# visinf/style-seqcvae

Measured on AMD Instinct MI355X. Metric: captions/sec (train step), higher is better.
Workload: dtype f32; 1 GPU; C2 train step: fwd+bwd+allreduce+clip+SGD, B=64/GPU, R=36, F=2048, L=20 (T=21), Z=128, V=10000, E=1000, H=1200, A=768, SENTIMENT_VAE=1; global_batch=64, parallelism=dp1

## Files before the change

### include/ssc.h

```cpp
#ifndef SSC_H
#define SSC_H

#include <stddef.h>
#include <stdint.h>

#ifdef __cplusplus
extern "C" {
#endif

#define SSC_OK 0
#define SSC_EINVAL (-1)
#define SSC_EALIGN (-2)
#define SSC_EHIP (-3)
#define SSC_EWORKSPACE (-4)

#define SSC_MAX_SEG 6

int ssc_version(void);
int ssc_last_hip_error(void);
const char* ssc_arch(void);

typedef struct {
  const float* A; const float* B;
  int lda, ldb, K;
// ... 72 lines not shown
  const float* c_prev; int ld_cprev;
  const float* c_new; int ld_cnew;
  float* dG;
  float* dc_prev; int ld_dcprev;
  float* dgsum;
  const float* slabsA; int nA; size_t strideA;
  const float* slabsB; int nB; size_t strideB;
} ssc_lstm_bwd_desc;
int ssc_lstm_bwd(const ssc_lstm_bwd_desc* d, void* stream);
int ssc_lstm_bwd_x(const ssc_lstm_bwd_desc* d, const float* x, int ldx, const float* w, int ldw, int K, void* stream);

int ssc_attn_logits(const float* q, int ldq, const float* pv, const float* wa, int G, int R, int A, int rows_per_image,
                    float* logits, void* stream);
int ssc_attn_fwd(const float* q, int ldq, const float* pv, const float* wa, const float* mask, const float* feats,
                 int G, int R, int A, int F, int rows_per_image, float* logits, float* alpha, float* att, int ldatt,
                 void* stream);

int ssc_attn_weights(const float* q, int ldq, const float* pv, const float* wa, const float* mask, int G, int R, int A,
                     int rows_per_image, float* logits, float* alpha, void* stream);

int ssc_attn_pool(const float* alpha, const float* x, int G, int R, int D, int rows_per_image, float* out, int ldo,
                  void* stream);
int ssc_attn_fwd_pool(const float* q, int ldq, const float* pv, const float* wa, const float* mask, const float* feats,
                      int G, int R, int A, int F, int rows_per_image, float* logits, float* alpha, float* att, int ldatt,
                      const float* obj, int D, float* pool, int ldpool, void* stream);

int ssc_attn_bwd(const float* datt, int lddatt, const float* q, int ldq, const float* pv, const float* wa,
                 const float* alpha, const float* feats, int G, int R, int A, int F, float* dq, int lddq,
                 float* dpv_acc, float* dwa_acc, float* scratch_dalpha, void* stream);
int ssc_attn_bwd_pool(const float* datt, int lddatt, const float* q, int ldq, const float* pv, const float* wa,
                      const float* alpha, const float* feats, int G, int R, int A, int F, float* dq, int lddq,
                      float* dpv_acc, float* dwa_acc, float* scratch_dalpha, const float* obj, int D, const float* dpool_a,
                      int lddpa, int Da, const float* dpool_b, int lddpb, void* stream);

typedef struct {
  int B, Z;
  const float* mulv; int ldmulv; int nslab; size_t slab_stride;
  const float* bmu; const float* blv;
  const float* eps; int ldeps;
  int kld_mode;
  const float* sent; float pm_scale; float prior_var;
  const float* w;
  float* mu; float* lv; float* z; int ldz;
  float* kld_acc;
  const float* pm; int ldpm;
} ssc_latent_fwd_desc;
int ssc_latent_fwd(const ssc_latent_fwd_desc* d, void* stream);

int ssc_latent_prior_sample(const float* eps, int ldeps, const float* sent, float pm_scale, float prior_var, int G, int Z,
                            float* z, int ldz, void* stream);

int ssc_latent_prior_sample_pm(const float* eps, int ldeps, const float* pm, int ldpm, const float* pv, int ldpv, const float* sent,
                               float pm_scale, float prior_var, int G, int Z, float* z, int ldz, void* stream);

typedef struct {
  int B, Z;
  const float* dz; int lddz;
  const float* eps; int ldeps;
  const float* mu; const float* lv; int ldz;
  int kld_mode; const float* sent; float pm_scale; float prior_var;
  const float* w; const float* gk;
  float* dmulv; int lddmulv;
  int nslab; size_t slab_stride;
  const float* pm; int ldpm;
  float* dpm; int lddpm;
} ssc_latent_bwd_desc;
// ... 389 lines not shown
```

### style-seqcvae_amd/csrc/attention.hip

```cpp
#include "ssc_common.h"

namespace {

constexpr int ATTN_RG = 8;
constexpr int ATTN_MAXA = 4096;
__global__ __launch_bounds__(256) void attn_logits_kernel(const float* __restrict__ q, int ldq, int nslab, size_t slab_stride,
                                                          float* __restrict__ q_out, int ldqo,
                                                          const float* __restrict__ pv, const float* __restrict__ wa,
                                                          int G, int R, int A, int rows_per_image,
                                                          float* __restrict__ logits, const int* __restrict__ rows,
                                                          const int* __restrict__ row_count) {
  __shared__ __attribute__((aligned(16))) float sq[ATTN_MAXA];
  const int groups = (R + ATTN_RG - 1) / ATTN_RG;
  int g = blockIdx.x / groups;
  const int grp = blockIdx.x - g * groups;
  if (rows) {
    if (g >= *row_count) return;
    g = rows[g];
  }
  const int tid = threadIdx.x, wave = tid >> 6, lane = tid & 63;
  const int img = g / rows_per_image;
  const float* qp = q + (size_t)g * ldq;
  const bool vec = ((A & 3) == 0) && ((ldq & 3) == 0) && ((ldqo & 3) == 0) && ((slab_stride & 3) == 0) && ssc_aligned16_dev(qp) &&
                   ssc_aligned16_dev(pv) && ssc_aligned16_dev(wa) && (!q_out || ssc_aligned16_dev(q_out));
// ... 181 lines not shown
  out[(size_t)g * ldo + d] = acc;
}

__global__ __launch_bounds__(256) void attn_dalpha_kernel(const float* __restrict__ datt, int lddatt,
                                                          const float* __restrict__ feats, int G, int R, int F,
                                                          float* __restrict__ dalpha, const float* __restrict__ obj, int D,
                                                          const float* __restrict__ dpa, int lddpa, int Da,
                                                          const float* __restrict__ dpb, int lddpb) {
  int wid = blockIdx.x * 4 + (threadIdx.x >> 6);
  int lane = threadIdx.x & 63;
  if (wid >= G * R) return;
  int g = wid / R;
  const float* dp = datt + (size_t)g * lddatt;
  const float* fp = feats + (size_t)wid * F;
  float s = 0.f;
  if (((F & 3) == 0) && ((lddatt & 3) == 0) && ssc_aligned16_dev(dp) && ssc_aligned16_dev(fp)) {
    for (int f = lane * 4; f < F; f += 256) {
      float4 a = *reinterpret_cast<const float4*>(dp + f);
      float4 b = *reinterpret_cast<const float4*>(fp + f);
      s += a.x * b.x + a.y * b.y + a.z * b.z + a.w * b.w;
    }
  } else {
    for (int f = lane; f < F; f += 64) s += dp[f] * fp[f];
  }
  if (obj) {
    const float* op = obj + (size_t)wid * D;
    for (int k = lane; k < D; k += 64)
      s += ((k < Da ? dpa[(size_t)g * lddpa + k] : 0.f) + (dpb ? dpb[(size_t)g * lddpb + k] : 0.f)) * op[k];
  }
  s = ssc_wave_sum(s);
  if (lane == 0) dalpha[wid] = s;
}

__global__ __launch_bounds__(256) void attn_bwd_apply_kernel(const float* __restrict__ q, int ldq,
                                                             const float* __restrict__ pv, const float* __restrict__ wa,
                                                             const float* __restrict__ alpha,
                                                             const float* __restrict__ dalpha, int G, int R, int A,
                                                             float* __restrict__ dq, int lddq, float* __restrict__ dpv_acc,
                                                             float* __restrict__ dwa_acc) {
  __shared__ float sdl[64 * MAXR_LANE];
  __shared__ float red[2][4][256];
  const int g = blockIdx.y, chunk = blockIdx.x, tid = threadIdx.x, lane = tid & 63, wave = tid >> 6;
  float c = 0.f;
  for (int r = lane; r < R; r += 64) c += alpha[(size_t)g * R + r] * dalpha[(size_t)g * R + r];
  c = ssc_wave_sum(c);
  if (wave == 0)
    for (int r = lane; r < R; r += 64) sdl[r] = alpha[(size_t)g * R + r] * (dalpha[(size_t)g * R + r] - c);
  __syncthreads();
  const int a0 = chunk * 256 + lane * 4;
  float dqa[4] = {0.f, 0.f, 0.f, 0.f}, dw[4] = {0.f, 0.f, 0.f, 0.f};
  const bool vec = ((A & 3) == 0) && ((ldq & 3) == 0) && ssc_aligned16_dev(q) && ssc_aligned16_dev(pv) &&
                   ssc_aligned16_dev(wa) && ssc_aligned16_dev(dpv_acc);
  if (vec) {
    if (a0 < A) {
      const float4 qv = *reinterpret_cast<const float4*>(q + (size_t)g * ldq + a0);
      const float4 wv = *reinterpret_cast<const float4*>(wa + a0);
      const float qa[4] = {qv.x, qv.y, qv.z, qv.w}, ww[4] = {wv.x, wv.y, wv.z, wv.w};
      for (int rb = wave; rb < R; rb += 4 * 5) {
        float4 p4[5], ac[5];
#pragma unroll
        for (int i = 0; i < 5; ++i) {
          const size_t off = ((size_t)g * R + min(rb + 4 * i, R - 1)) * A + a0;
          p4[i] = *reinterpret_cast<const float4*>(pv + off);
          ac[i] = *reinterpret_cast<const float4*>(dpv_acc + off);
        }
#pragma unroll
        for (int i = 0; i < 5; ++i) {
          const int r = rb + 4 * i;
          if (r < R) {
            const float pp[4] = {p4[i].x, p4[i].y, p4[i].z, p4[i].w};
            float dp[4];
            const float dl = sdl[r];
#pragma unroll
            for (int k = 0; k < 4; ++k) {
              float u = ssc_tanh_fast(qa[k] + pp[k]);
              dp[k] = dl * ww[k] * (1.f - u * u);
              dqa[k] += dp[k];
              dw[k] += dl * u;
            }
            float4 acc = ac[i];
            acc.x += dp[0]; acc.y += dp[1]; acc.z += dp[2]; acc.w += dp[3];
            *reinterpret_cast<float4*>(dpv_acc + ((size_t)g * R + r) * A + a0) = acc;
          }
        }
      }
    }
  } else {
    for (int k = 0; k < 4; ++k) {
      int a = chunk * 256 + k * 64 + lane;
      if (a >= A) continue;
      float qa = q[(size_t)g * ldq + a], w = wa[a];
      for (int r = wave; r < R; r += 4) {
        size_t off = ((size_t)g * R + r) * A + a;
        float u = ssc_tanh_fast(qa + pv[off]);
        float dl = sdl[r];
        float dpre = dl * w * (1.f - u * u);
        dpv_acc[off] += dpre;
        dqa[k] += dpre;
        dw[k] += dl * u;
      }
    }
  }
#pragma unroll
  for (int k = 0; k < 4; ++k) {
    red[0][wave][lane * 4 + k] = dqa[k];
    red[1][wave][lane * 4 + k] = dw[k];
  }
  __syncthreads();
  {
    float s0 = red[0][0][tid] + red[0][1][tid] + red[0][2][tid] + red[0][3][tid];
    float s1 = red[1][0][tid] + red[1][1][tid] + red[1][2][tid] + red[1][3][tid];
    int l = tid >> 2, k = tid & 3;
    int a = vec ? (chunk * 256 + l * 4 + k) : (chunk * 256 + k * 64 + l);
    if (a < A) {
      dq[(size_t)g * lddq + a] = s0;
      dwa_acc[(size_t)g * A + a] += s1;
    }
  }
}

}

extern "C" int ssc_attn_logits(const float* q, int ldq, const float* pv, const float* wa, int G, int R, int A,
                               int rows_per_image, float* logits, void* stream) {
  if (!q || !pv || !wa || !logits || G <= 0 || R <= 0 || A <= 0 || A > ATTN_MAXA || rows_per_image <= 0 || ldq < A) return SSC_EINVAL;
  SSC_LAUNCH(attn_logits_kernel, dim3(G * ssc_cdiv(R, ATTN_RG)), dim3(256), 0, (hipStream_t)stream, q, ldq, 1, (size_t)0,
                     (float*)nullptr, 0, pv, wa, G, R, A, rows_per_image, logits, (const int*)nullptr, (const int*)nullptr);
  SSC_CHECK_LAUNCH();
  return SSC_OK;
}

int ssc_attn_weights_rows(const float* q, int ldq, const float* pv, const float* wa, const float* mask, int G, int R, int A,
                          int rows_per_image, float* logits, float* alpha, const int* rows, const int* row_count, hipStream_t st) {
  if (!q || !pv || !wa || !mask || !alpha || !logits || !rows || !row_count || G <= 0 || R <= 0 || A <= 0 || A > ATTN_MAXA ||
      rows_per_image <= 0 || ldq < A || R > 64 * MAXR_LANE)
    return SSC_EINVAL;
  SSC_LAUNCH(attn_logits_kernel, dim3(G * ssc_cdiv(R, ATTN_RG)), dim3(256), 0, st, q, ldq, 1, (size_t)0, (float*)nullptr, 0, pv, wa,
             G, R, A, rows_per_image, logits, rows, row_count);
  SSC_CHECK_LAUNCH();
  SSC_LAUNCH(attn_apply_kernel, dim3(1, G), dim3(64), 0, st, logits, mask, (const float*)nullptr, G, R, 4, rows_per_image, alpha,
             (float*)nullptr, 0, (const float*)nullptr, 0, (float*)nullptr, 0);
  SSC_CHECK_LAUNCH();
  return SSC_OK;
}

extern "C" int ssc_attn_fwd(const float* q, int ldq, const float* pv, const float* wa, const float* mask,
                            const float* feats, int G, int R, int A, int F, int rows_per_image, float* logits,
                            float* alpha, float* att, int ldatt, void* stream) {
  if (!mask || !feats || !alpha || !att || !logits || F <= 0 || ldatt < F) return SSC_EINVAL;
  if (R > 64 * MAXR_LANE) return SSC_EINVAL;
  SSC_TRY(ssc_attn_logits(q, ldq, pv, wa, G, R, A, rows_per_image, logits, stream));
  SSC_LAUNCH(attn_apply_kernel, dim3(ssc_cdiv(F, 256), G), dim3(64), 0, (hipStream_t)stream, logits, mask, feats,
                     G, R, F, rows_per_image, alpha, att, ldatt, (const float*)nullptr, 0, (float*)nullptr, 0);
// ... 30 lines not shown
  SSC_LAUNCH(attn_pool_kernel, dim3(ssc_cdiv((D + 3) & ~3, 128), G), dim3(128), 0, (hipStream_t)stream, alpha, x, G, R, D, rows_per_image,
             out, ldo);
  SSC_CHECK_LAUNCH();
  return SSC_OK;
}

int ssc_attn_fwd_qslabs(const float* qslabs, int nslab, size_t slab_stride, float* q_out, int ldqo, const float* pv,
                        const float* wa, const float* mask, const float* feats, int G, int R, int A, int F,
                        int rows_per_image, float* logits, float* alpha, float* att, int ldatt, hipStream_t st,
                        const float* obj, int D, float* pool, int ldpool) {
  if (!qslabs || nslab < 1 || !q_out || !pv || !wa || !mask || !feats || !alpha || !att || !logits) return SSC_EINVAL;
  if (obj && (!pool || D <= 0 || ldpool < D)) return SSC_EINVAL;
  if (G <= 0 || R <= 0 || A <= 0 || A > ATTN_MAXA || F <= 0 || ldatt < F || ldqo < A || R > 64 * MAXR_LANE) return SSC_EINVAL;
  SSC_LAUNCH(attn_logits_kernel, dim3(G * ssc_cdiv(R, ATTN_RG)), dim3(256), 0, st, qslabs, A, nslab, slab_stride, q_out,
                     ldqo, pv, wa, G, R, A, rows_per_image, logits, (const int*)nullptr, (const int*)nullptr);
  SSC_CHECK_LAUNCH();
  SSC_LAUNCH(attn_apply_kernel, dim3(ssc_cdiv(F, 256) + (obj ? ssc_cdiv(ldpool, 256) : 0), G), dim3(64), 0, st, logits, mask, feats,
             G, R, F, rows_per_image, alpha, att, ldatt, obj, D, pool, ldpool);
  SSC_CHECK_LAUNCH();
  return SSC_OK;
}

extern "C" int ssc_attn_bwd(const float* datt, int lddatt, const float* q, int ldq, const float* pv, const float* wa,
                            const float* alpha, const float* feats, int G, int R, int A, int F, float* dq, int lddq,
                            float* dpv_acc, float* dwa_acc, float* scratch_dalpha, void* stream) {
  return ssc_attn_bwd_pool(datt, lddatt, q, ldq, pv, wa, alpha, feats, G, R, A, F, dq, lddq, dpv_acc, dwa_acc, scratch_dalpha,
                           nullptr, 0, nullptr, 0, 0, nullptr, 0, stream);
}

extern "C" int ssc_attn_bwd_pool(const float* datt, int lddatt, const float* q, int ldq, const float* pv, const float* wa,
                                 const float* alpha, const float* feats, int G, int R, int A, int F, float* dq, int lddq,
                                 float* dpv_acc, float* dwa_acc, float* scratch_dalpha, const float* obj, int D,
                                 const float* dpool_a, int lddpa, int Da, const float* dpool_b, int lddpb, void* stream) {
  if (!datt || !q || !pv || !wa || !alpha || !feats || !dq || !dpv_acc || !dwa_acc || !scratch_dalpha) return SSC_EINVAL;
  if (G <= 0 || R <= 0 || A <= 0 || F <= 0 || R > 64 * MAXR_LANE || lddatt < F || ldq < A || lddq < A) return SSC_EINVAL;
  if (obj && (!dpool_a || D <= 0 || Da < 0 || Da > D || lddpa < Da || (dpool_b && lddpb < D))) return SSC_EINVAL;
  SSC_LAUNCH(attn_dalpha_kernel, dim3(ssc_cdiv(G * R, 4)), dim3(256), 0, (hipStream_t)stream, datt, lddatt, feats,
                     G, R, F, scratch_dalpha, obj, D, dpool_a, lddpa, Da, dpool_b, lddpb);
  SSC_CHECK_LAUNCH();
  SSC_LAUNCH(attn_bwd_apply_kernel, dim3(ssc_cdiv(A, 256), G), dim3(256), 0, (hipStream_t)stream, q, ldq, pv, wa,
                     alpha, scratch_dalpha, G, R, A, dq, lddq, dpv_acc, dwa_acc);
  SSC_CHECK_LAUNCH();
  return SSC_OK;
}
```

### style-seqcvae_amd/csrc/gemm.hip

```cpp
#include <stdio.h>
#include <stdlib.h>
#include <string.h>

#include "ssc_common.h"
#include "ssc_debug.h"

typedef float f32x16 __attribute__((ext_vector_type(16)));

namespace {

constexpr int BM = 64, BN = 64, BK = 32;
constexpr int KC_LD = BK + 4;

struct KSeg {
  const float* A;
  const float* B;
  int lda, ldb, K, nsteps;
  int avec, bvec;
  const float* A16;
  const float* B16;
  int lda16, ldb16;
};

struct KArgs {
// ... 2221 lines not shown
extern "C" int ssc_prof_collect(float* out, int max_records) {
  if (!out || !g_prof) return 0;
  if (hipDeviceSynchronize() != hipSuccess) return SSC_EHIP;
  int n = g_prof_n < max_records ? g_prof_n : max_records;
  for (int i = 0; i < n; ++i) {
    float ms = 0.f;
    (void)hipEventElapsedTime(&ms, g_prof[i].e0, g_prof[i].e1);
    float* o = out + (size_t)i * 8;
    g_prof[i].bytes = g_prof[i].flops = 0.0;
    for (int q = 0; q < g_prof[i].nmem; ++q) {
      const ProfMember& m = g_prof[i].mem[q];
      double M = m.M, K = m.K;
      if (m.slot_m >= 0 && g_prof_counts[m.slot_m] >= 0 && g_prof_counts[m.slot_m] < m.M) M = g_prof_counts[m.slot_m];
      if (m.slot_k >= 0 && g_prof_counts[m.slot_k] >= 0 && g_prof_counts[m.slot_k] < m.K) K = g_prof_counts[m.slot_k];
      g_prof[i].bytes += 4.0 * (K * m.N + M * K + M * m.N);
      g_prof[i].flops += 2.0 * M * m.N * K;
    }
    o[0] = (float)g_prof[i].kind; o[1] = (float)g_prof[i].M; o[2] = (float)g_prof[i].N; o[3] = (float)g_prof[i].K;
    o[4] = (float)g_prof[i].splits; o[5] = ms; o[6] = (float)g_prof[i].bytes; o[7] = (float)g_prof[i].flops;
  }
  g_prof_n = 0;
  g_prof_slots = 0;
  return n;
}

extern "C" int ssc_set_gemm_mode(int mode) {
  int prev = gemm_mode();
  if (mode == 0 || mode == 1) g_gemm_mode = mode;
  return prev;
}

extern int ssc_g_dec_att_table, ssc_g_dec_dedup, ssc_g_beam_reg, ssc_g_dec_ungathered, ssc_g_dec_parts, ssc_g_dec_planes;
extern int ssc_g_img_mfma;
extern int ssc_g_dw_one_flush;
namespace {
struct DebugKey { const char* name; int* var; };
const DebugKey g_debug_keys[] = {
    {"large_form", &g_x3b},
    {"x3w_skinny", &g_x3w_skinny},
    {"store_wt", &g_store_wt},
    {"tile_gm", &g_tile_gm},
    {"dw_one_flush", &ssc_g_dw_one_flush},
    {"dec_dedup", &ssc_g_dec_dedup},
    {"beam_reg", &ssc_g_beam_reg},
    {"img_mfma", &ssc_g_img_mfma},
    {"dec_ungathered", &ssc_g_dec_ungathered},
    {"dec_planes", &ssc_g_dec_planes},
    {"dec_parts", &ssc_g_dec_parts},
    {"dec_att_table", &ssc_g_dec_att_table},
    {"f16_npw", &g_f16_npw},
    {"gemm_f16", &g_gemm_f16},
};
}

extern "C" int ssc_debug_set(const char* key, int value) {
  if (!key) return SSC_EINVAL;
  for (const DebugKey& k : g_debug_keys)
    if (!strcmp(k.name, key)) { *k.var = value; return SSC_OK; }
  return SSC_EINVAL;
}
extern "C" int ssc_debug_get(const char* key, int* value) {
  if (!key || !value) return SSC_EINVAL;
  for (const DebugKey& k : g_debug_keys)
    if (!strcmp(k.name, key)) { *value = *k.var; return SSC_OK; }
  return SSC_EINVAL;
}

#ifdef SSC_X3W_STAMP
extern "C" int ssc_debug_stamp_setup(void* buf, int wg) {
  if (hipMemcpyToSymbol(HIP_SYMBOL(g_stamp_ptr), &buf, sizeof(buf)) != hipSuccess) return SSC_EHIP;
  if (hipMemcpyToSymbol(HIP_SYMBOL(g_stamp_wg), &wg, sizeof(wg)) != hipSuccess) return SSC_EHIP;
  return SSC_OK;
}
#endif
```

### style-seqcvae_amd/csrc/sequence.hip

```cpp
#include <cstdlib>
#include <initializer_list>

#include "ssc_common.h"
#include "ssc_debug.h"

namespace {

inline size_t r4(size_t x) { return (x + 3) & ~(size_t)3; }

struct Layout {
  int B, R, L, T;
  int V, E, H, A, F, Z, S, tied;
  int Ep, Hp, Ap, Fp, Zp, Vp, H4, XW;
  int D, Dp, SC, NX;
  size_t wc_e, wc_d, pool, dpm;
  size_t total = 0;
  size_t act;
  size_t live;
  size_t tok, w, nvalid, sent_all, wcol_e, wcol_d, mask, avg, pv, emb, ga_static, ga_avg;
  size_t h1, c1, he, ce, hd, cd, gates_a, gates_e, gates_d, q, attn_logits, alpha, att, mu, lv, z, mulv;
  size_t slabs, slab_floats, logits, lse, proj;
  size_t nllw0, nll;
  size_t sl_q, sl_mulv, sl_gh1, sl_ghd, sl_ghd2, sl_ghe, sl_dqw, sl_dhe, sl_dz, small_floats, wsum_att, wsum_dec, wz;
  size_t sl_ga, sl_ge, sl_gd, gate_floats;
// ... 41 lines not shown
  l.mulv = l.take((size_t)B * 2 * l.Z);
  size_t skinny = (size_t)33 * B * l.H4;
  size_t full = (size_t)16 * 1024 * 1024;
  l.slab_floats = skinny > full ? skinny : full;
  l.slabs = l.take(l.slab_floats);
  {
    size_t w = (size_t)(l.Hp > l.Ap ? l.Hp : l.Ap);
    if ((size_t)2 * l.Z > w) w = (size_t)2 * l.Z;
    l.small_floats = (size_t)40 * B * w;
    l.sl_q = l.take(l.small_floats); l.sl_mulv = l.take(l.small_floats);
    l.sl_gh1 = l.take(l.small_floats); l.sl_ghd = l.take(l.small_floats); l.sl_ghe = l.take(l.small_floats);
    l.sl_ghd2 = l.take(l.small_floats);
    l.sl_dqw = l.take(l.small_floats); l.sl_dhe = l.take(l.small_floats); l.sl_dz = l.take(l.small_floats);
  }
  l.gate_floats = (size_t)34 * B * l.H4;
  l.sl_ga = l.take(l.gate_floats); l.sl_ge = l.take(l.gate_floats); l.sl_gd = l.take(l.gate_floats);
  l.wsum_att = l.take((size_t)l.H4 * l.Hp);
  l.wsum_dec = l.take((size_t)l.H4 * l.Hp);
  l.wz = l.take((size_t)l.H4 * l.Zp);
  l.wc_e = l.take((size_t)l.H4 * l.Dp); l.wc_d = l.take((size_t)l.H4 * l.Dp);
  l.pool = l.take(TB * l.Dp); l.dpm = l.take((size_t)B * l.Dp);
  l.logits = l.take(TB * l.Vp);
  l.lse = l.take(2 * TB);
  l.proj = l.take(l.tied ? TB * l.Ep : 0);
  l.dhdv = l.take(TB * l.Hp);
  l.dga = l.take(TB * l.H4); l.dge = l.take(TB * l.H4); l.dgd = l.take(TB * l.H4);
  l.dga_sum = l.take((size_t)B * l.H4);
  l.g_h1 = l.take((size_t)B * l.Hp); l.g_c1 = l.take((size_t)B * l.Hp);
  l.g_he = l.take((size_t)B * l.Hp); l.g_ce = l.take((size_t)B * l.Hp);
  l.g_cd = l.take((size_t)B * l.Hp);
  l.dz = l.take((size_t)B * l.Zp);
  l.dmulv = l.take(TB * 2 * l.Z);
  l.dx = l.take((size_t)B * l.XW);
  l.dalpha = l.take((size_t)B * R);
  l.dq = l.take(TB * l.Ap);
  l.dpv = l.take((size_t)B * R * l.A);
  l.dwa = l.take((size_t)B * l.A);
  l.demb = l.take(TB * l.Ep);
  l.dproj = l.take(l.tied ? TB * l.Ep : 0);
  l.nllw0 = l.take(TB);
  l.nll = l.take(B);
  return l;
}

struct Seg {
  const float* A; int lda;
  const float* B; int ldb;
  int K;
};

struct Ctx {
  hipStream_t st;
  float* slabs;
  size_t slab_floats;
  const int* act_count = nullptr;
  const int* act_rows = nullptr;
  const int* live_count = nullptr;
  const int* live_rows = nullptr;
};

void fill_desc(ssc_gemm_desc& d, bool a_kc, bool b_kc, std::initializer_list<Seg> segs, int M, int N) {
  d = ssc_gemm_desc{};
  int i = 0;
  for (const Seg& s : segs) {
    if (s.K <= 0) continue;
    d.seg[i].A = s.A; d.seg[i].lda = s.lda; d.seg[i].B = s.B; d.seg[i].ldb = s.ldb; d.seg[i].K = s.K;
    ++i;
// ... 434 lines not shown
    }
#pragma unroll
    for (int u = 0; u < 4; ++u) acc += (r0 + 16 * u < rows) ? d4[u] * x4[u] : 0.f;
  }
  part[rl][nl] = acc;
  __syncthreads();
  if (rl == 0 && blockIdx.x * 64 + nl < N) {
    float t = part[0][nl];
    for (int i = 1; i < 16; ++i) t += part[i][nl];
    dW[(size_t)(v0 + j) * ldw + n] = t;
  }
}
int head_tail_rows(const float* dlog, int ldl, const float* Wt, int ldw, int v0, int V, int rows, int N, float* out, int ldo, hipStream_t st) {
  const int nt = V - v0;
  if (nt <= 0) return SSC_OK;
  SSC_LAUNCH(head_tail_rows_kernel, dim3(ssc_cdiv(N, 256), rows), dim3(256), 0, st, dlog, ldl, Wt, ldw, v0, nt, N, out, ldo);
  SSC_CHECK_LAUNCH();
  return SSC_OK;
}
int head_tail_dw(const float* dlog, int ldl, const float* X, int ldx, int v0, int V, int rows, int N, float* dW, int ldw, hipStream_t st) {
  const int nt = V - v0;
  if (nt <= 0) return SSC_OK;
  SSC_LAUNCH(head_tail_dw_kernel, dim3(ssc_cdiv(N, 64), nt), dim3(1024), 0, st, dlog, ldl, X, ldx, rows, v0, N, dW, ldw);
  SSC_CHECK_LAUNCH();
  return SSC_OK;
}
__global__ void repeat_kernel(const float* __restrict__ src, int n, int reps, float* __restrict__ dst) {
  int i = blockIdx.x * blockDim.x + threadIdx.x;
  if (i < n * reps) dst[i] = src[i % n];
}
}

int ssc_g_dw_one_flush = ssc_env_int("SSC_DW_ONE_FLUSH", 1);

static int train_bwd_impl(const ssc_model_cfg* cfg, const ssc_params* p, const ssc_batch* bt, void* workspace,
                          size_t workspace_bytes, const float* gl, const float* gk, const ssc_params* g, void* stream,
                          unsigned phases) {
  SscGemmModeScope mode_scope(cfg);
  SSC_TRY(check_cfg(cfg, p, bt));
  if (!workspace || !gl || !gk || !g) return SSC_EINVAL;
  const Layout l = make_layout(cfg, bt->B, bt->R, bt->L);
  if (workspace_bytes < l.total * sizeof(float)) return SSC_EWORKSPACE;
  float* W = (float*)workspace;
  hipStream_t st = (hipStream_t)stream;
  Ctx c{st, W + l.slabs, l.slab_floats};
  const int B = l.B, R = l.R, T = l.T, E = l.E, H = l.H, A = l.A, F = l.F, Z = l.Z, S = l.S, V = l.V, H4 = l.H4;
  const int TB = T * B, XW = l.XW;
  int64_t* tok = (int64_t*)(W + l.tok);
  const size_t sH = (size_t)B * l.Hp;
  const float* hd_all = W + l.hd + sH;
  const bool one_flush = ssc_g_dw_one_flush && (phases & (128u | 4u | 8u)) == (128u | 4u | 8u);
  DwBatch dwq;
  c.act_count = (const int*)(W + l.act); c.act_rows = c.act_count + 4;
  c.live_count = (const int*)(W + l.live); c.live_rows = c.live_count + 4;

  if (phases & (1u | 16u)) {
  SSC_TRY(ssc_ce_bwd_smooth(W + l.logits, l.Vp, tok + B, W + l.w, W + l.nvalid, W + l.lse, gl, T, B, V, cfg->label_smoothing, st));
  const float* dlog = W + l.logits;
  {
    FillList f;
    f.add(W + l.dhdv, (size_t)TB * l.Hp);
    if (cfg->tied) f.add(W + l.dproj, (size_t)TB * l.Ep);
    for (size_t off : {l.g_c1, l.g_ce, l.g_cd}) f.add(W + off, sH);
    f.add(W + l.dx, (size_t)B * XW);
    f.add(W + l.dpv, (size_t)B * R * A);
    f.add(W + l.dwa, (size_t)B * A);
    f.add(W + l.dga_sum, (size_t)B * H4);
    SSC_TRY(fill_many(f, 0.f, st));
  }
  const int V4 = V >= 8 ? (V & ~3) : V;
  if (cfg->tied) {
    float* dP = W + l.dproj;
    SSC_TRY(gemm_rows(c, false, {{dlog, l.Vp, p->emb, p->ld_emb, V4}}, TB, E, dP, l.Ep));
    SSC_TRY(head_tail_rows(dlog, l.Vp, p->emb, p->ld_emb, V4, V, TB, E, dP, l.Ep, st));
    SSC_TRY(ssc_tanh_bwd(dP, l.Ep, W + l.proj, l.Ep, TB, E, st));
    SSC_TRY(gemm_rows(c, false, {{dP, l.Ep, p->proj_w, p->ld_proj_w, E}}, TB, H, W + l.dhdv, l.Hp));
    if (g->proj_w) {
      SSC_TRY(queue_dw(c, dwq, dP, l.Ep, hd_all, l.Hp, TB, E, H, g->proj_w, g->ld_proj_w));
      if (!one_flush) SSC_TRY(flush_dw(c, dwq));
    }
    if (g->proj_b) SSC_TRY(ssc_colsum2(dP, l.Ep, TB, E, nullptr, g->proj_b, 1, nullptr, 0, c.slabs, st));
  } else {
    SSC_TRY(gemm_rows(c, false, {{dlog, l.Vp, p->out_w, p->ld_out_w, V4}}, TB, H, W + l.dhdv, l.Hp));
    SSC_TRY(head_tail_rows(dlog, l.Vp, p->out_w, p->ld_out_w, V4, V, TB, H, W + l.dhdv, l.Hp, st));
    if (g->out_w) {
      SSC_TRY(queue_dw(c, dwq, dlog, l.Vp, hd_all, l.Hp, TB, V4, H, g->out_w, g->ld_out_w));
      if (!one_flush) SSC_TRY(flush_dw(c, dwq));
      SSC_TRY(head_tail_dw(dlog, l.Vp, hd_all, l.Hp, V4, V, TB, H, g->out_w, g->ld_out_w, st));
    }
    if (g->out_b) SSC_TRY(ssc_colsum2(dlog, l.Vp, TB, V, nullptr, g->out_b, 1, nullptr, 0, c.slabs, st));
  }
  }

  if (phases & (1u | 32u)) {
  float* dx = W + l.dx;
  int n_gh1 = 0, n_ghd = 0, n_ghd2 = 0, n_ghe = 0;
  const bool fc_adjacent_b = (p->fc_lv_w == p->fc_mean_w + (size_t)Z * p->ld_fc_mean_w) && p->ld_fc_lv_w == p->ld_fc_mean_w;
  const size_t sBH = (size_t)B * H;
  const int NX = l.NX;
  const size_t sBX = (size_t)B * NX;

  if (g_loop.on) { (void)hipEventRecord(g_loop.e[2], st); }
  for (int t = T - 1; t >= 0; --t) {
    float* dgd = W + l.dgd + (size_t)t * B * H4;
    float* dge = W + l.dge + (size_t)t * B * H4;
    float* dga = W + l.dga + (size_t)t * B * H4;
    float* dmulv = W + l.dmulv + (size_t)t * B * 2 * Z;
    float* dq = W + l.dq + (size_t)t * B * l.Ap;
    int ns = 0, n_dxd = 0, n_dxe = 0;
    {
      ssc_lstm_bwd_desc d{};
      d.B = B; d.H = H;
      d.dh = dx + F + H; d.ld_dh = XW;
      d.dh2 = W + l.dhdv + (size_t)t * B * l.Hp; d.ld_dh2 = l.Hp;
      d.slabsA = W + l.sl_ghd; d.nA = n_ghd; d.strideA = sBH;
      d.slabsB = W + l.sl_ghd2; d.nB = n_ghd2; d.strideB = sBH;
      d.dc_in = W + l.g_cd; d.ld_dcin = l.Hp;
      d.gates = W + l.gates_d + (size_t)t * B * H4;
      d.c_prev = W + l.cd + t * sH; d.ld_cprev = l.Hp;
      d.c_new = W + l.cd + (t + 1) * sH; d.ld_cnew = l.Hp;
      d.dG = dgd; d.dc_prev = W + l.g_cd; d.ld_dcprev = l.Hp;
      SSC_TRY(ssc_lstm_bwd(&d, st));
    }
    {
      ssc_gemm_desc d3[3];
      fill_desc(d3[0], true, false, {{dgd, H4, W + l.wz, l.Zp, H4}}, B, l.Zp);
      fill_desc(d3[1], true, false, {{dgd, H4, p->dec_w_ih, p->ld_dec_w_ih, H4}}, B, NX);
      fill_desc(d3[2], true, false, {{dgd, H4, p->dec_w_hh, p->ld_dec_w_hh, H4}}, B, H);
      const ssc_gemm_desc* dp[3] = {&d3[0], &d3[1], &d3[2]};
      float* regions[3] = {W + l.sl_dz, c.slabs, W + l.sl_ghd2};
      const size_t caps[3] = {l.small_floats, c.slab_floats / 2, l.small_floats};
      int ns3[3] = {0, 0, 0};
      SSC_TRY(ssc_gemm_slabs_group(dp, t > 0 ? 3 : 2, regions, caps, ns3, st));
// ... 14 lines not shown
    }
    {
      ssc_lstm_bwd_desc d{};
      d.B = B; d.H = H;
      d.slabsA = W + l.sl_ghe; d.nA = n_ghe; d.strideA = sBH;
      d.dc_in = W + l.g_ce; d.ld_dcin = l.Hp;
      d.gates = W + l.gates_e + (size_t)t * B * H4;
      d.c_prev = W + l.ce + t * sH; d.ld_cprev = l.Hp;
      d.c_new = W + l.ce + (t + 1) * sH; d.ld_cnew = l.Hp;
      d.dG = dge; d.dc_prev = W + l.g_ce; d.ld_dcprev = l.Hp;
      if (fc_adjacent_b && 2 * Z <= 768) {
        SSC_TRY(ssc_lstm_bwd_x(&d, dmulv, 2 * Z, p->fc_mean_w, p->ld_fc_mean_w, 2 * Z, st));
      } else {
        SSC_TRY(gemm_to_slabs(c, W + l.sl_dhe, l.small_floats, true, false,
                              {{dmulv, 2 * Z, p->fc_mean_w, p->ld_fc_mean_w, Z}, {dmulv + Z, 2 * Z, p->fc_lv_w, p->ld_fc_lv_w, Z}}, B, H,
                              &ns));
        d.slabsB = W + l.sl_dhe; d.nB = ns; d.strideB = sBH;
        SSC_TRY(ssc_lstm_bwd(&d, st));
      }
    }
    {
      ssc_gemm_desc d2[2];
      fill_desc(d2[0], true, false, {{dge, H4, p->enc_w_ih, p->ld_enc_w_ih, H4}}, B, NX);
      fill_desc(d2[1], true, false, {{dge, H4, p->enc_w_hh, p->ld_enc_w_hh, H4}}, B, H);
      const ssc_gemm_desc* dp[2] = {&d2[0], &d2[1]};
      float* regions[2] = {c.slabs + (size_t)n_dxd * sBX, W + l.sl_ghe};
      const size_t caps[2] = {c.slab_floats - (size_t)n_dxd * sBX, l.small_floats};
      int ns2[2] = {0, 0};
      SSC_TRY(ssc_gemm_slabs_group(dp, t > 0 ? 2 : 1, regions, caps, ns2, st));
      n_dxe = ns2[0]; n_ghe = ns2[1];
    }
    SSC_TRY(ssc_reduce_slabs(c.slabs, n_dxd + n_dxe, sBX, B, NX, dx, XW, nullptr, 0, st));
    SSC_TRY(ssc_attn_bwd_pool(dx, XW, W + l.q + (size_t)t * B * l.Ap, l.Ap, W + l.pv, p->wa, W + l.alpha + (size_t)t * B * R,
                              bt->feats, B, R, A, F, dq, l.Ap, W + l.dpv, W + l.dwa, W + l.dalpha, l.D ? bt->obj_atts : nullptr, l.D,
                              dx + F + 2 * H, XW, l.SC, W + l.dpm, l.Dp, st));
    {
      ssc_lstm_bwd_desc d{};
      d.B = B; d.H = H;
      d.dh = dx + F; d.ld_dh = XW;
      d.slabsA = W + l.sl_gh1; d.nA = n_gh1; d.strideA = sBH;
      d.dc_in = W + l.g_c1; d.ld_dcin = l.Hp;
      d.gates = W + l.gates_a + (size_t)t * B * H4;
      d.c_prev = W + l.c1 + t * sH; d.ld_cprev = l.Hp;
      d.c_new = W + l.c1 + (t + 1) * sH; d.ld_cnew = l.Hp;
      d.dG = dga; d.dc_prev = W + l.g_c1; d.ld_dcprev = l.Hp;
      d.dgsum = W + l.dga_sum;
      const bool fused_q = A <= 768;
      if (fused_q) {
        SSC_TRY(ssc_lstm_bwd_x(&d, dq, l.Ap, p->wq, p->ld_wq, A, st));
      } else {
        SSC_TRY(gemm_to_slabs(c, W + l.sl_dqw, l.small_floats, true, false, {{dq, l.Ap, p->wq, p->ld_wq, A}}, B, H, &ns));
        d.slabsB = W + l.sl_dqw; d.nB = ns; d.strideB = sBH;
        SSC_TRY(ssc_lstm_bwd(&d, st));
      }
    }
    if (t > 0) {
      const float* wr = p->att_w_ih + E + F;
      ssc_gemm_desc d2[2];
      fill_desc(d2[0], true, false, {{dga, H4, W + l.wsum_att, l.Hp, H4}}, B, H);
      fill_desc(d2[1], true, false, {{dga, H4, wr + H, p->ld_att_w_ih, H4}}, B, H);
      const ssc_gemm_desc* dp[2] = {&d2[0], &d2[1]};
      float* regions[2] = {W + l.sl_gh1, W + l.sl_ghd};
      const size_t caps[2] = {l.small_floats, l.small_floats};
      int ns2[2] = {0, 0};
      SSC_TRY(ssc_gemm_slabs_group(dp, 2, regions, caps, ns2, st));
      n_gh1 = ns2[0]; n_ghd = ns2[1];
    }
  }

  if (g_loop.on) { (void)hipEventRecord(g_loop.e[3], st); g_loop.bwd = true; }

  if (S == 1 && !l.D) {
    SSC_LAUNCH(repeat_kernel, dim3(ssc_cdiv(TB, 256)), dim3(256), 0, st, bt->sentiment, B, T, W + l.sent_all);
    SSC_CHECK_LAUNCH();
  }
  }

  const int zcol = F + 2 * H + S;
  const float* dga = W + l.dga; const float* dge = W + l.dge; const float* dgd = W + l.dgd;
  const float* h1_prev = W + l.h1; const float* h1_new = W + l.h1 + sH;
  const float* hd_prev = W + l.hd; const float* he_prev = W + l.he; const float* he_new = W + l.he + sH;
  const float* att = W + l.att;
  if (phases & 64u) {
  if (g->emb && !cfg->tied) {
    SSC_TRY(ssc_fill(W + l.demb, (size_t)TB * l.Ep, 0.f, st));
    SSC_TRY(gemm_rows(c, false, {{dga, H4, p->att_w_ih, p->ld_att_w_ih, H4}}, TB, E, W + l.demb, l.Ep, nullptr, true));
    if (hipMemset2DAsync(g->emb, (size_t)g->ld_emb * sizeof(float), 0, (size_t)E * sizeof(float), V, st) != hipSuccess)
      return SSC_EHIP;
    SSC_TRY(ssc_embed_scatter_add(g->emb, g->ld_emb, tok, TB, E, W + l.demb, l.Ep, cfg->pad, st));
  }
  }
  auto queue_att = [&](DwBatch& q) -> int {
    if (g->att_w_ih) {
      float* gw = g->att_w_ih; int ld = g->ld_att_w_ih;
      SSC_TRY(queue_dw(c, q, dga, H4, W + l.emb, l.Ep, TB, H4, E, gw, ld));
      SSC_TRY(queue_dw(c, q, dga, H4, h1_prev, l.Hp, TB, H4, H, gw + E + F, ld));
      SSC_TRY(queue_dw(c, q, dga, H4, hd_prev, l.Hp, TB, H4, H, gw + E + F + H, ld));
    } else if (g->att_w_hh) {
      SSC_TRY(queue_dw(c, q, dga, H4, h1_prev, l.Hp, TB, H4, H, g->att_w_hh, g->ld_att_w_hh));
    }
    if (g->wq) SSC_TRY(queue_dw(c, q, W + l.dq, l.Ap, h1_new, l.Hp, TB, A, H, g->wq, g->ld_wq));
    return SSC_OK;
  };
  auto queue_enc = [&](DwBatch& q) -> int {
// ... 135 lines not shown
```

### style-seqcvae_amd/ssc_runtime/lib.py

```python
import ctypes as C
import os

_HERE = os.path.dirname(os.path.abspath(__file__))
DEBUG_ENV = os.environ.get("SSC_DEBUG", "") == "1"
LIB_PATH = (DEBUG_ENV and os.environ.get("SSC_LIB_PATH")) or os.path.join(os.path.dirname(_HERE), "libssc_hip.so")
SSC_MAX_SEG = 6

c_float_p = C.POINTER(C.c_float)
c_i64_p = C.POINTER(C.c_int64)
vp = C.c_void_p


class SscError(RuntimeError):
    CODES = {-1: "SSC_EINVAL", -2: "SSC_EALIGN", -3: "SSC_EHIP", -4: "SSC_EWORKSPACE"}

    def __init__(self, fn, rc, hip=0):
        super().__init__(f"{fn} failed: {self.CODES.get(rc, rc)}" + (f" (hipError {hip})" if rc == -3 else ""))
        self.rc = rc


class GemmSeg(C.Structure):
    _fields_ = [("A", vp), ("B", vp), ("lda", C.c_int), ("ldb", C.c_int), ("K", C.c_int),
                ("A16", vp), ("B16", vp), ("lda16", C.c_int), ("ldb16", C.c_int)]

# ... 162 lines not shown
                ("loss_scale", C.c_double), ("kld_scale", C.c_double), ("caps", vp), ("lengths", vp), ("reward", vp),
                ("advantage", vp), ("gl", vp), ("gk", vp), ("stats", vp)]


_i, _f, _sz = C.c_int, C.c_float, C.c_size_t
SYMBOLS = {
    "ssc_version": (_i, []),
    "ssc_last_hip_error": (_i, []),
    "ssc_arch": (C.c_char_p, []),
    "ssc_gemm": (_i, [C.POINTER(GemmDesc), vp]),
    "ssc_gemm_dw_group": (_i, [C.POINTER(C.POINTER(GemmDesc)), _i, vp]),
    "ssc_gemm_auto_splits": (_i, [_i, _i, _i]),
    "ssc_pow2_scale": (_i, [vp, _sz, _i, _sz, _i, vp, _i, vp, vp]),
    "ssc_split_f16": (_i, [vp, _i, _i, _i, vp, vp, _i, vp, vp, vp]),
    "ssc_decode_planes_ld": (_i, [vp]),
    "ssc_set_gemm_mode": (_i, [_i]),
    "ssc_feat_prep": (_i, [vp, _i, _i, _i, vp, vp, vp]),
    "ssc_prep_tokens": (_i, [vp, _i, _i, _i, _i, vp, vp, vp, vp]),
    "ssc_embed_gather": (_i, [vp, _i, vp, _i, _i, vp, _i, vp]),
    "ssc_embed_scatter_add": (_i, [vp, _i, vp, _i, _i, vp, _i, _i, vp]),
    "ssc_lstm_fwd": (_i, [C.POINTER(LstmFwdDesc), vp]),
    "ssc_lstm_fwd_z": (_i, [C.POINTER(LstmFwdDesc), vp, _i, vp, _i, _i, vp]),
    "ssc_lstm_fwd_p": (_i, [C.POINTER(LstmFwdDesc), vp, _i, _i, vp, vp]),
    "ssc_lstm_fwd_img": (_i, [C.POINTER(LstmFwdDesc), vp, _i, vp, _i, _i, vp]),
    "ssc_lstm_bwd_x": (_i, [C.POINTER(LstmBwdDesc), vp, _i, vp, _i, _i, vp]),
    "ssc_lstm_bwd": (_i, [C.POINTER(LstmBwdDesc), vp]),
    "ssc_attn_logits": (_i, [vp, _i, vp, vp, _i, _i, _i, _i, vp, vp]),
    "ssc_attn_fwd": (_i, [vp, _i, vp, vp, vp, vp, _i, _i, _i, _i, _i, vp, vp, vp, _i, vp]),
    "ssc_attn_weights": (_i, [vp, _i, vp, vp, vp, _i, _i, _i, _i, vp, vp, vp]),
    "ssc_attn_pool": (_i, [vp, vp, _i, _i, _i, _i, vp, _i, vp]),
    "ssc_attn_fwd_pool": (_i, [vp, _i, vp, vp, vp, vp, _i, _i, _i, _i, _i, vp, vp, vp, _i, vp, _i, vp, _i, vp]),
    "ssc_attn_bwd_pool": (_i, [vp, _i, vp, _i, vp, vp, vp, vp, _i, _i, _i, _i, vp, _i, vp, vp, vp, vp, _i, vp, _i, _i, vp, _i, vp]),
    "ssc_attn_bwd": (_i, [vp, _i, vp, _i, vp, vp, vp, vp, _i, _i, _i, _i, vp, _i, vp, vp, vp, vp]),
    "ssc_latent_fwd": (_i, [C.POINTER(LatentFwdDesc), vp]),
    "ssc_latent_prior_sample": (_i, [vp, _i, vp, _f, _f, _i, _i, vp, _i, vp]),
    "ssc_latent_prior_sample_pm": (_i, [vp, _i, vp, _i, vp, _i, vp, _f, _f, _i, _i, vp, _i, vp]),
    "ssc_latent_bwd": (_i, [C.POINTER(LatentBwdDesc), vp]),
    "ssc_ce_fwd": (_i, [vp, _i, vp, vp, vp, _i, _i, _i, vp, vp, vp]),
    "ssc_ce_bwd": (_i, [vp, _i, vp, vp, vp, vp, vp, _i, _i, _i, vp]),
    "ssc_ce_fwd_smooth": (_i, [vp, _i, vp, vp, vp, _i, _i, _i, _f, vp, vp, vp, vp]),
    "ssc_ce_bwd_smooth": (_i, [vp, _i, vp, vp, vp, vp, vp, _i, _i, _i, _f, vp]),
    "ssc_log_softmax": (_i, [vp, _i, _i, _i, vp, _i, vp]),
    "ssc_colsum": (_i, [vp, _i, _i, _i, vp, vp, _i, _i, vp]),
    "ssc_colsum2": (_i, [vp, _i, _i, _i, vp, vp, _i, vp, _i, vp, vp]),
    "ssc_copy_strided": (_i, [vp, _sz, _i, vp, vp]),
    "ssc_bias_tanh": (_i, [vp, _i, _i, _i, vp, vp]),
    "ssc_tanh_bwd": (_i, [vp, _i, vp, _i, _i, _i, vp]),
    "ssc_fill": (_i, [vp, _sz, _f, vp]),
    "ssc_sq_norm": (_i, [vp, _sz, vp, vp, vp]),
    "ssc_sgd_step": (_i, [vp, vp, vp, _sz, vp, _f, _f, _f, _f, _f, _i, vp]),
    "ssc_adam_step": (_i, [vp, vp, vp, vp, _sz, vp, _f, _f, _f, _f, _f, _f, _f, _i, _i, vp]),
    "ssc_train_workspace_bytes": (_sz, [C.POINTER(ModelCfg), _i, _i, _i]),
    "ssc_train_fwd": (_i, [C.POINTER(ModelCfg), C.POINTER(Params), C.POINTER(Batch), vp, _sz, vp, vp, vp]),
    "ssc_train_bwd": (_i, [C.POINTER(ModelCfg), C.POINTER(Params), C.POINTER(Batch), vp, _sz, vp, vp, C.POINTER(Params), vp]),
    "ssc_train_bwd_phases": (_i, [C.POINTER(ModelCfg), C.POINTER(Params), C.POINTER(Batch), vp, _sz, vp, vp, C.POINTER(Params),
                                  C.c_uint, vp]),
    "ssc_train_workspace_view": (vp, [C.POINTER(ModelCfg), _i, _i, _i, vp, _i, C.POINTER(C.c_int)]),
    "ssc_xgmi_enable_peer": (_i, [_i]),
    "ssc_xgmi_ipc_export": (_i, [vp, vp, C.POINTER(C.c_size_t)]),
    "ssc_xgmi_ipc_open": (_i, [vp, C.POINTER(vp)]),
    "ssc_xgmi_ipc_close": (_i, [vp]),
    "ssc_xgmi_peek": (_i, [vp, vp, _sz]),
    "ssc_xgmi_allreduce": (_i, [C.POINTER(XgmiComm), _sz, _sz, C.c_uint, C.c_uint, vp, vp]),
    "ssc_decode_image_bytes": (_sz, [C.POINTER(ModelCfg), _i, _i]),
    "ssc_decode_prepare": (_i, [C.POINTER(ModelCfg), C.POINTER(Params), vp, _i, _i, vp, _sz, vp]),
    "ssc_decode_prepare_from": (_i, [C.POINTER(ModelCfg), C.POINTER(Params), vp, _i, _i, vp, _sz, vp, _i, _i, vp]),
# ... 115 lines not shown
```

Measured before the change: 8002 captions/s.

## Accumulate attention dpv once after backward loop instead of per timestep

In the per-timestep attention backward pass, the kernel no longer reads and writes the B*R*A dpv accumulator. Instead, dalpha is stored for every timestep, and a new kernel sums the dpv contributions over all T steps in one pass after the loop. This cuts read-modify-write traffic on a roughly 64*36*768 buffer at every step. In exchange, tanh is recomputed in the new kernel, dalpha scratch grows to T*B*R, and the non-accumulating apply kernel prefetches pv before the reduction. The behaviour is controlled by an env flag that defaults to on.

```diff
diff --git a/include/ssc.h b/include/ssc.h
--- a/include/ssc.h
+++ b/include/ssc.h
@@ -128,6 +128,8 @@
                       const float* alpha, const float* feats, int G, int R, int A, int F, float* dq, int lddq,
                       float* dpv_acc, float* dwa_acc, float* scratch_dalpha, const float* obj, int D, const float* dpool_a,
                       int lddpa, int Da, const float* dpool_b, int lddpb, void* stream);
+int ssc_attn_dpv_sum(const float* q, int ldq, const float* pv, const float* wa, const float* alpha, const float* dalpha, int T,
+                     int G, int R, int A, float* dpv, void* stream);
 
 typedef struct {
   int B, Z;
diff --git a/style-seqcvae_amd/csrc/attention.hip b/style-seqcvae_amd/csrc/attention.hip
--- a/style-seqcvae_amd/csrc/attention.hip
+++ b/style-seqcvae_amd/csrc/attention.hip
@@ -237,6 +237,15 @@
   if (lane == 0) dalpha[wid] = s;
 }
 
+__device__ __forceinline__ float attn_bwd_c(const float* __restrict__ alpha, const float* __restrict__ dalpha, int R, int lane) {
+  float c = 0.f;
+  for (int r = lane; r < R; r += 64) c += alpha[r] * dalpha[r];
+  return ssc_wave_sum(c);
+}
+__device__ __forceinline__ float attn_bwd_dl(float alpha, float dalpha, float c) { return alpha * (dalpha - c); }
+__device__ __forceinline__ float attn_bwd_dpre(float dl, float w, float u) { return dl * w * (1.f - u * u); }
+
+template <bool ACC>
 __global__ __launch_bounds__(256) void attn_bwd_apply_kernel(const float* __restrict__ q, int ldq,
                                                              const float* __restrict__ pv, const float* __restrict__ wa,
                                                              const float* __restrict__ alpha,
@@ -246,31 +255,34 @@
   __shared__ float sdl[64 * MAXR_LANE];
   __shared__ float red[2][4][256];
   const int g = blockIdx.y, chunk = blockIdx.x, tid = threadIdx.x, lane = tid & 63, wave = tid >> 6;
-  float c = 0.f;
-  for (int r = lane; r < R; r += 64) c += alpha[(size_t)g * R + r] * dalpha[(size_t)g * R + r];
-  c = ssc_wave_sum(c);
-  if (wave == 0)
-    for (int r = lane; r < R; r += 64) sdl[r] = alpha[(size_t)g * R + r] * (dalpha[(size_t)g * R + r] - c);
-  __syncthreads();
+  constexpr int NB = ACC ? 5 : 10;
   const int a0 = chunk * 256 + lane * 4;
-  float dqa[4] = {0.f, 0.f, 0.f, 0.f}, dw[4] = {0.f, 0.f, 0.f, 0.f};
   const bool vec = ((A & 3) == 0) && ((ldq & 3) == 0) && ssc_aligned16_dev(q) && ssc_aligned16_dev(pv) &&
                    ssc_aligned16_dev(wa) && ssc_aligned16_dev(dpv_acc);
+  float4 p4[NB], ac[ACC ? NB : 1];
+  auto request = [&](int rb) __attribute__((always_inline)) {
+#pragma unroll
+    for (int i = 0; i < NB; ++i) {
+      const size_t off = ((size_t)g * R + min(rb + 4 * i, R - 1)) * A + a0;
+      p4[i] = *reinterpret_cast<const float4*>(pv + off);
+      if constexpr (ACC) ac[i] = *reinterpret_cast<const float4*>(dpv_acc + off);
+    }
+  };
+  if constexpr (!ACC) { if (vec && a0 < A) request(wave); }
+  const float c = attn_bwd_c(alpha + (size_t)g * R, dalpha + (size_t)g * R, R, lane);
+  if (wave == 0)
+    for (int r = lane; r < R; r += 64) sdl[r] = attn_bwd_dl(alpha[(size_t)g * R + r], dalpha[(size_t)g * R + r], c);
+  __syncthreads();
+  float dqa[4] = {0.f, 0.f, 0.f, 0.f}, dw[4] = {0.f, 0.f, 0.f, 0.f};
   if (vec) {
     if (a0 < A) {
       const float4 qv = *reinterpret_cast<const float4*>(q + (size_t)g * ldq + a0);
       const float4 wv = *reinterpret_cast<const float4*>(wa + a0);
       const float qa[4] = {qv.x, qv.y, qv.z, qv.w}, ww[4] = {wv.x, wv.y, wv.z, wv.w};
-      for (int rb = wave; rb < R; rb += 4 * 5) {
-        float4 p4[5], ac[5];
-#pragma unroll
-        for (int i = 0; i < 5; ++i) {
-          const size_t off = ((size_t)g * R + min(rb + 4 * i, R - 1)) * A + a0;
-          p4[i] = *reinterpret_cast<const float4*>(pv + off);
-          ac[i] = *reinterpret_cast<const float4*>(dpv_acc + off);
-        }
-#pragma unroll
-        for (int i = 0; i < 5; ++i) {
+      for (int rb = wave; rb < R; rb += 4 * NB) {
+        if (ACC || rb != wave) request(rb);
+#pragma unroll
+        for (int i = 0; i < NB; ++i) {
           const int r = rb + 4 * i;
           if (r < R) {
             const float pp[4] = {p4[i].x, p4[i].y, p4[i].z, p4[i].w};
@@ -279,13 +291,15 @@
 #pragma unroll
             for (int k = 0; k < 4; ++k) {
               float u = ssc_tanh_fast(qa[k] + pp[k]);
-              dp[k] = dl * ww[k] * (1.f - u * u);
+              dp[k] = attn_bwd_dpre(dl, ww[k], u);
               dqa[k] += dp[k];
               dw[k] += dl * u;
             }
-            float4 acc = ac[i];
-            acc.x += dp[0]; acc.y += dp[1]; acc.z += dp[2]; acc.w += dp[3];
-            *reinterpret_cast<float4*>(dpv_acc + ((size_t)g * R + r) * A + a0) = acc;
+            if constexpr (ACC) {
+              float4 acc = ac[i];
+              acc.x += dp[0]; acc.y += dp[1]; acc.z += dp[2]; acc.w += dp[3];
+              *reinterpret_cast<float4*>(dpv_acc + ((size_t)g * R + r) * A + a0) = acc;
+            }
           }
         }
       }
@@ -299,8 +313,8 @@
         size_t off = ((size_t)g * R + r) * A + a;
         float u = ssc_tanh_fast(qa + pv[off]);
         float dl = sdl[r];
-        float dpre = dl * w * (1.f - u * u);
-        dpv_acc[off] += dpre;
+        float dpre = attn_bwd_dpre(dl, w, u);
+        if constexpr (ACC) dpv_acc[off] += dpre;
         dqa[k] += dpre;
         dw[k] += dl * u;
       }
@@ -324,6 +338,53 @@
   }
 }
 
+__global__ __launch_bounds__(256) void attn_dpv_sum_kernel(const float* __restrict__ q, int ldq, const float* __restrict__ pv,
+                                                           const float* __restrict__ wa, const float* __restrict__ alpha,
+                                                           const float* __restrict__ dalpha, int T, int G, int R, int A,
+                                                           float* __restrict__ dpv) {
+  extern __shared__ float dpv_sdl[];
+  const int g = blockIdx.y, chunk = blockIdx.x, tid = threadIdx.x, lane = tid & 63, wave = tid >> 6;
+  const int r0 = blockIdx.z * 4;
+  for (int t = wave; t < T; t += 4) {
+    const size_t row = ((size_t)t * G + g) * R;
+    const float c = attn_bwd_c(alpha + row, dalpha + row, R, lane);
+    if (lane < 4) dpv_sdl[t * 4 + lane] = r0 + lane < R ? attn_bwd_dl(alpha[row + r0 + lane], dalpha[row + r0 + lane], c) : 0.f;
+  }
+  __syncthreads();
+  const int r = r0 + wave;
+  if (r >= R) return;
+  const size_t off = ((size_t)g * R + r) * A;
+  const bool vec = ((A & 3) == 0) && ((ldq & 3) == 0) && ssc_aligned16_dev(q) && ssc_aligned16_dev(pv) &&
+                   ssc_aligned16_dev(wa) && ssc_aligned16_dev(dpv);
+  if (vec) {
+    const int a0 = chunk * 256 + lane * 4;
+    if (a0 >= A) return;
+    const float4 pv4 = *reinterpret_cast<const float4*>(pv + off + a0);
+    const float4 wv = *reinterpret_cast<const float4*>(wa + a0);
+    const float pp[4] = {pv4.x, pv4.y, pv4.z, pv4.w}, ww[4] = {wv.x, wv.y, wv.z, wv.w};
+    float acc[4] = {0.f, 0.f, 0.f, 0.f};
+#pragma unroll 4
+    for (int t = T - 1; t >= 0; --t) {
+      const float4 qv = *reinterpret_cast<const float4*>(q + ((size_t)t * G + g) * ldq + a0);
+      const float qa[4] = {qv.x, qv.y, qv.z, qv.w};
+      const float dl = dpv_sdl[t * 4 + wave];
+#pragma unroll
+      for (int k = 0; k < 4; ++k) acc[k] += attn_bwd_dpre(dl, ww[k], ssc_tanh_fast(qa[k] + pp[k]));
+    }
+    *reinterpret_cast<float4*>(dpv + off + a0) = make_float4(acc[0], acc[1], acc[2], acc[3]);
+  } else {
+    for (int k = 0; k < 4; ++k) {
+      const int a = chunk * 256 + k * 64 + lane;
+      if (a >= A) continue;
+      const float p = pv[off + a], w = wa[a];
+      float acc = 0.f;
+      for (int t = T - 1; t >= 0; --t)
+        acc += attn_bwd_dpre(dpv_sdl[t * 4 + wave], w, ssc_tanh_fast(q[((size_t)t * G + g) * ldq + a] + p));
+      dpv[off + a] = acc;
+    }
+  }
+}
+
 }
 
 extern "C" int ssc_attn_logits(const float* q, int ldq, const float* pv, const float* wa, int G, int R, int A,
@@ -420,14 +481,28 @@
                                  const float* alpha, const float* feats, int G, int R, int A, int F, float* dq, int lddq,
                                  float* dpv_acc, float* dwa_acc, float* scratch_dalpha, const float* obj, int D,
                                  const float* dpool_a, int lddpa, int Da, const float* dpool_b, int lddpb, void* stream) {
-  if (!datt || !q || !pv || !wa || !alpha || !feats || !dq || !dpv_acc || !dwa_acc || !scratch_dalpha) return SSC_EINVAL;
+  if (!datt || !q || !pv || !wa || !alpha || !feats || !dq || !dwa_acc || !scratch_dalpha) return SSC_EINVAL;
   if (G <= 0 || R <= 0 || A <= 0 || F <= 0 || R > 64 * MAXR_LANE || lddatt < F || ldq < A || lddq < A) return SSC_EINVAL;
   if (obj && (!dpool_a || D <= 0 || Da < 0 || Da > D || lddpa < Da || (dpool_b && lddpb < D))) return SSC_EINVAL;
   SSC_LAUNCH(attn_dalpha_kernel, dim3(ssc_cdiv(G * R, 4)), dim3(256), 0, (hipStream_t)stream, datt, lddatt, feats,
                      G, R, F, scratch_dalpha, obj, D, dpool_a, lddpa, Da, dpool_b, lddpb);
   SSC_CHECK_LAUNCH();
-  SSC_LAUNCH(attn_bwd_apply_kernel, dim3(ssc_cdiv(A, 256), G), dim3(256), 0, (hipStream_t)stream, q, ldq, pv, wa,
-                     alpha, scratch_dalpha, G, R, A, dq, lddq, dpv_acc, dwa_acc);
-  SSC_CHECK_LAUNCH();
-  return SSC_OK;
-}
+  if (dpv_acc)
+    SSC_LAUNCH(attn_bwd_apply_kernel<true>, dim3(ssc_cdiv(A, 256), G), dim3(256), 0, (hipStream_t)stream, q, ldq, pv, wa, alpha,
+               scratch_dalpha, G, R, A, dq, lddq, dpv_acc, dwa_acc);
+  else
+    SSC_LAUNCH(attn_bwd_apply_kernel<false>, dim3(ssc_cdiv(A, 256), G), dim3(256), 0, (hipStream_t)stream, q, ldq, pv, wa, alpha,
+               scratch_dalpha, G, R, A, dq, lddq, dpv_acc, dwa_acc);
+  SSC_CHECK_LAUNCH();
+  return SSC_OK;
+}
+
+extern "C" int ssc_attn_dpv_sum(const float* q, int ldq, const float* pv, const float* wa, const float* alpha, const float* dalpha,
+                                int T, int G, int R, int A, float* dpv, void* stream) {
+  if (!q || !pv || !wa || !alpha || !dalpha || !dpv) return SSC_EINVAL;
+  if (T <= 0 || T > 4096 || G <= 0 || R <= 0 || A <= 0 || R > 64 * MAXR_LANE || ldq < A) return SSC_EINVAL;
+  SSC_LAUNCH(attn_dpv_sum_kernel, dim3(ssc_cdiv(A, 256), G, ssc_cdiv(R, 4)), dim3(256), (size_t)T * 4 * sizeof(float),
+             (hipStream_t)stream, q, ldq, pv, wa, alpha, dalpha, T, G, R, A, dpv);
+  SSC_CHECK_LAUNCH();
+  return SSC_OK;
+}
diff --git a/style-seqcvae_amd/csrc/gemm.hip b/style-seqcvae_amd/csrc/gemm.hip
--- a/style-seqcvae_amd/csrc/gemm.hip
+++ b/style-seqcvae_amd/csrc/gemm.hip
@@ -2277,7 +2277,7 @@
 
 extern int ssc_g_dec_att_table, ssc_g_dec_dedup, ssc_g_beam_reg, ssc_g_dec_ungathered, ssc_g_dec_parts, ssc_g_dec_planes;
 extern int ssc_g_img_mfma;
-extern int ssc_g_dw_one_flush;
+extern int ssc_g_dw_one_flush, ssc_g_dpv_once;
 namespace {
 struct DebugKey { const char* name; int* var; };
 const DebugKey g_debug_keys[] = {
@@ -2286,6 +2286,7 @@
     {"store_wt", &g_store_wt},
     {"tile_gm", &g_tile_gm},
     {"dw_one_flush", &ssc_g_dw_one_flush},
+    {"dpv_once", &ssc_g_dpv_once},
     {"dec_dedup", &ssc_g_dec_dedup},
     {"beam_reg", &ssc_g_beam_reg},
     {"img_mfma", &ssc_g_img_mfma},
diff --git a/style-seqcvae_amd/csrc/sequence.hip b/style-seqcvae_amd/csrc/sequence.hip
--- a/style-seqcvae_amd/csrc/sequence.hip
+++ b/style-seqcvae_amd/csrc/sequence.hip
@@ -97,7 +97,7 @@
   l.dz = l.take((size_t)B * l.Zp);
   l.dmulv = l.take(TB * 2 * l.Z);
   l.dx = l.take((size_t)B * l.XW);
-  l.dalpha = l.take((size_t)B * R);
+  l.dalpha = l.take(TB * R);
   l.dq = l.take(TB * l.Ap);
   l.dpv = l.take((size_t)B * R * l.A);
   l.dwa = l.take((size_t)B * l.A);
@@ -598,6 +598,7 @@
 }
 
 int ssc_g_dw_one_flush = ssc_env_int("SSC_DW_ONE_FLUSH", 1);
+int ssc_g_dpv_once = ssc_env_int("SSC_DPV_ONCE", 1);
 
 static int train_bwd_impl(const ssc_model_cfg* cfg, const ssc_params* p, const ssc_batch* bt, void* workspace,
                           size_t workspace_bytes, const float* gl, const float* gk, const ssc_params* g, void* stream,
@@ -629,7 +630,7 @@
     if (cfg->tied) f.add(W + l.dproj, (size_t)TB * l.Ep);
     for (size_t off : {l.g_c1, l.g_ce, l.g_cd}) f.add(W + off, sH);
     f.add(W + l.dx, (size_t)B * XW);
-    f.add(W + l.dpv, (size_t)B * R * A);
+    if (!ssc_g_dpv_once) f.add(W + l.dpv, (size_t)B * R * A);
     f.add(W + l.dwa, (size_t)B * A);
     f.add(W + l.dga_sum, (size_t)B * H4);
     SSC_TRY(fill_many(f, 0.f, st));
@@ -665,6 +666,7 @@
   const size_t sBH = (size_t)B * H;
   const int NX = l.NX;
   const size_t sBX = (size_t)B * NX;
+  const bool dpv_once = ssc_g_dpv_once != 0;
 
   if (g_loop.on) { (void)hipEventRecord(g_loop.e[2], st); }
   for (int t = T - 1; t >= 0; --t) {
@@ -745,7 +747,8 @@
     }
     SSC_TRY(ssc_reduce_slabs(c.slabs, n_dxd + n_dxe, sBX, B, NX, dx, XW, nullptr, 0, st));
     SSC_TRY(ssc_attn_bwd_pool(dx, XW, W + l.q + (size_t)t * B * l.Ap, l.Ap, W + l.pv, p->wa, W + l.alpha + (size_t)t * B * R,
-                              bt->feats, B, R, A, F, dq, l.Ap, W + l.dpv, W + l.dwa, W + l.dalpha, l.D ? bt->obj_atts : nullptr, l.D,
+                              bt->feats, B, R, A, F, dq, l.Ap, dpv_once ? nullptr : W + l.dpv, W + l.dwa,
+                              W + l.dalpha + (size_t)t * B * R, l.D ? bt->obj_atts : nullptr, l.D,
                               dx + F + 2 * H, XW, l.SC, W + l.dpm, l.Dp, st));
     {
       ssc_lstm_bwd_desc d{};
@@ -781,8 +784,9 @@
     }
   }
 
+  if (dpv_once) SSC_TRY(ssc_attn_dpv_sum(W + l.q, l.Ap, W + l.pv, p->wa, W + l.alpha, W + l.dalpha, T, B, R, A, W + l.dpv, st));
+
   if (g_loop.on) { (void)hipEventRecord(g_loop.e[3], st); g_loop.bwd = true; }
-
   if (S == 1 && !l.D) {
     SSC_LAUNCH(repeat_kernel, dim3(ssc_cdiv(TB, 256)), dim3(256), 0, st, bt->sentiment, B, T, W + l.sent_all);
     SSC_CHECK_LAUNCH();
diff --git a/style-seqcvae_amd/ssc_runtime/lib.py b/style-seqcvae_amd/ssc_runtime/lib.py
--- a/style-seqcvae_amd/ssc_runtime/lib.py
+++ b/style-seqcvae_amd/ssc_runtime/lib.py
@@ -218,6 +218,7 @@
     "ssc_attn_fwd_pool": (_i, [vp, _i, vp, vp, vp, vp, _i, _i, _i, _i, _i, vp, vp, vp, _i, vp, _i, vp, _i, vp]),
     "ssc_attn_bwd_pool": (_i, [vp, _i, vp, _i, vp, vp, vp, vp, _i, _i, _i, _i, vp, _i, vp, vp, vp, vp, _i, vp, _i, _i, vp, _i, vp]),
     "ssc_attn_bwd": (_i, [vp, _i, vp, _i, vp, vp, vp, vp, _i, _i, _i, _i, vp, _i, vp, vp, vp, vp]),
+    "ssc_attn_dpv_sum": (_i, [vp, _i, vp, vp, vp, vp, _i, _i, _i, _i, vp, vp]),
     "ssc_latent_fwd": (_i, [C.POINTER(LatentFwdDesc), vp]),
     "ssc_latent_prior_sample": (_i, [vp, _i, vp, _f, _f, _i, _i, vp, _i, vp]),
     "ssc_latent_prior_sample_pm": (_i, [vp, _i, vp, _i, vp, _i, vp, _f, _f, _i, _i, vp, _i, vp]),
```

Result: no change. 8047 captions/s, median of 6 (+0.6%).
